# corenel/pytorch-glow

Measured on AMD Instinct MI355X. Metric: images/sec full Glow fwd+logdet, 64x64x3 L=3 K=32, 1/2/4/8 GPU, higher is better.
Workload: dtype f32 (2xf16 split operands, fp32 accumulate); 1 GPU; CelebA 64x64x3 Glow L=3 K=32 hidden=512 affine+invconv, fwd+logdet, batch 64/GPU (BASELINE configs[1]); global_batch=64, parallelism=dp1, repack_every_step=True

## Files before the change

pytorch-glow_amd/csrc/pack.hip:

```cpp
#include <algorithm>

#include "kernels.h"
#include "conv_mfma.h"
#include "sh.h"
#include "lu_wave.h"

namespace glowhip {

__device__ __forceinline__ size_t align_up_dev(size_t v, size_t a) { return (v + a - 1) / a * a; }

__device__ __forceinline__ void pack_scales(const ScaleJob& j, char* packed, int bx, int nbx) {
    float* scale = (float*)(packed + j.scale_off);
    float* inv = j.has_inv ? (float*)(packed + j.inv_off) : nullptr;
    for (int i = bx * 256 + threadIdx.x; i < j.n; i += nbx * 256) {
        const float l3 = j.logs[i] * LOGSCALE;
        scale[i] = expf(l3);
        if (inv) inv[i] = expf(-l3);
    }
}
__global__ void __launch_bounds__(256) k_pack_scales_batched(const ScaleJob* __restrict__ jobs, char* packed) {
    pack_scales(jobs[blockIdx.y], packed, blockIdx.x, gridDim.x);
}

__device__ __forceinline__ void repack_legacy(const RepackJob& j, char* packed, int bx, int nbx) {
    float* out = (float*)(packed + j.out_off);
    if (j.kind == REPACK_WIDE) {
        const long total = (long)j.Kpad * j.Cout;
        for (long e = (long)bx * 256 + threadIdx.x; e < total; e += (long)nbx * 256) {
            const int k = (int)(e / j.Cout), o = (int)(e - (long)k * j.Cout);
            out[e] = (k < j.K) ? j.w[(long)o * j.K + k] : 0.f;
        }
    } else if (j.kind == REPACK_FIRST) {
        const long total = (long)9 * j.Cin * j.Cout;
        for (long e = (long)bx * 256 + threadIdx.x; e < total; e += (long)nbx * 256) {
            const int o = (int)(e % j.Cout);
            const int k = (int)(e / j.Cout);
            const int chunk = k / 54, r = k - chunk * 54;
            const int tap = r / 6, cl = r - tap * 6;
            const int ci = chunk * 6 + cl;
            const float wv = j.transposed ? j.w[((long)ci * j.Cout + o) * 9 + (8 - tap)] : j.w[((long)o * j.Cin + ci) * 9 + tap];
            out[e] = j.fold_logs ? wv * expf(j.fold_logs[o] * LOGSCALE) : wv;
        }
        for (long o = (long)bx * 256 + threadIdx.x; o < j.Cout; o += (long)nbx * 256)
            out[total + o] = j.fold_logs ? j.fold_bias[o] * expf(j.fold_logs[o] * LOGSCALE) : 0.f;
    } else {
        for (long e = (long)bx * 256 + threadIdx.x; e < j.total; e += (long)nbx * 256) {
            const int i = (int)(e & 15), kq = (int)((e >> 4) & 3);
            long t = e >> 6;
            const int mt = (int)(t % j.MT); t /= j.MT;
            const int tap = (int)(t % 9); t /= 9;
            const int c4 = (int)(t % (TAIL_CK / 4));
            const int chunk = (int)(t / (TAIL_CK / 4));
            const int ci = chunk * TAIL_CK + c4 * 4 + kq;
            const int o = tail_row_channel(mt * 16 + i, j.Cout, j.paired);
            out[e] = (o >= 0 && ci < j.Cin)
                         ? (j.transposed ? j.w[((long)ci * j.Cout + o) * 9 + (8 - tap)] : j.w[((long)o * j.Cin + ci) * 9 + tap])
                         : 0.f;
        }
    }
}
__global__ void __launch_bounds__(256) k_repack_batched(const RepackJob* __restrict__ jobs, char* packed) {
    const RepackJob j = jobs[blockIdx.y];
    if (j.kind >= REPACK_SH2_GEMM) return;
    repack_legacy(j, packed, blockIdx.x, gridDim.x);
}

__device__ __forceinline__ const float* repack_src(const RepackJob& j, const char* packed) {
    return j.w ? j.w : reinterpret_cast<const float*>(packed + j.w_off);
}

template <int KIND>
__device__ __forceinline__ void repack_sh2_rows(const RepackJob& j, char* packed, int bx, int nbx) {
    const float* jw = repack_src(j, packed);
    const int lane = threadIdx.x & 63, r8 = lane & 7, gl = lane >> 3;
    const int M = KIND == REPACK_SH2_TAIL ? j.Kpad : j.Cout;
    const int Kp = KIND == REPACK_SH2_FIRST ? j.K * 8 : j.Cin;
    const int ngroups = Kp / 8;
    _Float16* oh = (_Float16*)(packed + j.out_off);
    float* rowscale = (float*)(packed + j.out_off + (size_t)2 * Kp * M * sizeof(_Float16));
    float* rbias = rowscale + M;
    const int nchunk = (j.Cin + 7) / 8;
    for (int r0 = (bx * 4 + (threadIdx.x >> 6)) * 8; r0 < M; r0 += nbx * 32) {
        const int r = r0 + r8;
        const bool rv = r < M;
        float fold = 1.f;
        if (rv && KIND != REPACK_SH2_TAIL && j.fold_logs) fold = expf(j.fold_logs[r] * LOGSCALE);
        auto group = [&](int gi, float (&v)[8]) {
#pragma unroll
            for (int k8 = 0; k8 < 8; ++k8) v[k8] = 0.f;
            if (!rv || gi >= ngroups) return;
            if (KIND == REPACK_SH2_GEMM) {
                const float* src = jw + (long)r * j.Cin + (j.kperm ? sh2_kperm_src(gi * 8) : gi * 8);
                const int h2o = j.kperm ? 8 : 4;
                if ((j.Cin & 3) == 0) {
                    const f32x4_t a = *reinterpret_cast<const f32x4_t*>(src), b = *reinterpret_cast<const f32x4_t*>(src + h2o);
#pragma unroll
                    for (int k8 = 0; k8 < 4; ++k8) { v[k8] = a[k8] * fold; v[4 + k8] = b[k8] * fold; }
                } else {
#pragma unroll
                    for (int k8 = 0; k8 < 8; ++k8) v[k8] = src[(k8 & 3) + (k8 >> 2) * h2o] * fold;
                }
            } else if (KIND == REPACK_SH2_FIRST) {
                const int ch = gi / 9, tap = gi - ch * 9;
                if (ch < nchunk) {
#pragma unroll
                    for (int k8 = 0; k8 < 8; ++k8)
                        if (ch * 8 + k8 < j.Cin) v[k8] = jw[((long)r * j.Cin + ch * 8 + k8) * 9 + tap] * fold;
                }
            } else if (r < 9 * j.Cout) {
                const int tap = r / j.Cout, co = r - tap * j.Cout;
#pragma unroll
                for (int k8 = 0; k8 < 8; ++k8) v[k8] = jw[((long)co * j.Cin + gi * 8 + k8) * 9 + tap];
            }
        };
        float mx = 0.f;
        for (int gi = gl; gi < ngroups; gi += 8) {
            float v[8];
            group(gi, v);
#pragma unroll
            for (int k8 = 0; k8 < 8; ++k8) mx = fmaxf(mx, fabsf(v[k8]));
        }
        mx = fmaxf(mx, __shfl_xor(mx, 8, 64));
        mx = fmaxf(mx, __shfl_xor(mx, 16, 64));
        mx = fmaxf(mx, __shfl_xor(mx, 32, 64));
        int e = 0;
        if (mx > 0.f && mx < 3.0e38f) {
            int ex;
            (void)frexpf(mx, &ex);
            e = 13 - ex;
            e = e > 100 ? 100 : (e < -100 ? -100 : e);
        }
        const float up = ldexpf(1.f, e);
        for (int gi = gl; gi < ngroups; gi += 8) {
            float v[8];
            group(gi, v);
            h8 hi, lo;
#pragma unroll
            for (int k8 = 0; k8 < 8; ++k8) {
                _Float16 a, b;
                sh2_split(v[k8] * up, a, b);
                hi[k8] = a; lo[k8] = b;
            }
            if (rv) {
                *reinterpret_cast<h8*>(oh + ((long)gi * M + r) * 8) = hi;
                *reinterpret_cast<h8*>(oh + ((long)(ngroups + gi) * M + r) * 8) = lo;
            }
        }
        if (gl == 0 && rv) {
            if (KIND == REPACK_SH2_TAIL) {
                rowscale[r] = ldexpf(1.f, -e) * SH2_ACT_INV;
                rbias[r] = 0.f;
            } else {
                rowscale[r] = ldexpf(1.f, -e);
                rbias[r] = (j.fold_bias ? j.fold_bias[r] * fold : 0.f) * SH2_ACT_SCALE;
            }
        }
    }
}

__device__ __forceinline__ void load_brick(const float* src, int nk, bool valid, float (&b)[72]) {
#pragma unroll
    for (int i = 0; i < 72; ++i) b[i] = 0.f;
    if (!valid) return;
    const int count = nk * 9;
    if (nk == 8 && ((size_t)src & 15) == 0) {
#pragma unroll
        for (int i = 0; i < 18; ++i) {
            const f32x4_t v = reinterpret_cast<const f32x4_t*>(src)[i];
#pragma unroll
            for (int q = 0; q < 4; ++q) b[i * 4 + q] = v[q];
        }
    } else if ((count & 1) == 0 && ((size_t)src & 7) == 0) {
#pragma unroll
        for (int i = 0; i < 36; ++i)
            if (2 * i < count) {
                const f32x2_t v = reinterpret_cast<const f32x2_t*>(src)[i];
                b[2 * i] = v[0]; b[2 * i + 1] = v[1];
            }
    } else {
#pragma unroll
        for (int i = 0; i < 72; ++i)
            if (i < count) b[i] = src[i];
    }
}

__device__ __forceinline__ int sh2_row_exponent(float mx) {
    int e = 0;
    if (mx > 0.f && mx < 3.0e38f) {
        int ex;
        (void)frexpf(mx, &ex);
        e = 13 - ex;
        e = e > 100 ? 100 : (e < -100 ? -100 : e);
    }
    return e;
}

__device__ __forceinline__ void brick_emit(const float (&b)[72], int tap, float mul, h8& hi, h8& lo) {
#pragma unroll
    for (int k8 = 0; k8 < 8; ++k8) {
        _Float16 x, y;
        sh2_split(b[k8 * 9 + tap] * mul, x, y);
        hi[k8] = x; lo[k8] = y;
    }
}

__device__ __forceinline__ void repack_sh2_first(const RepackJob& j, char* packed, int bx, int nbx) {
    const int M = j.Cout, G = j.K, Kp = G * 8;
    _Float16* oh = (_Float16*)(packed + j.out_off);
    float* rowscale = (float*)(packed + j.out_off + (size_t)2 * Kp * M * sizeof(_Float16));
    float* rbias = rowscale + M;
    const int nchunk = (j.Cin + 7) / 8;
    for (int r = bx * 256 + threadIdx.x; r < M; r += nbx * 256) {
        const float fold = j.fold_logs ? expf(j.fold_logs[r] * LOGSCALE) : 1.f;
        const float* row = repack_src(j, packed) + (long)r * j.Cin * 9;
        float mx = 0.f;
        for (int ch = 0; ch < nchunk; ++ch) {
            float b[72];
            load_brick(row + ch * 72, min(8, j.Cin - ch * 8), true, b);
#pragma unroll
            for (int i = 0; i < 72; ++i) mx = fmaxf(mx, fabsf(b[i] * fold));
        }
        const int e = sh2_row_exponent(mx);
        const float up = ldexpf(1.f, e);
        for (int ch = 0; ch < nchunk; ++ch) {
            float b[72];
            load_brick(row + ch * 72, min(8, j.Cin - ch * 8), true, b);
#pragma unroll
            for (int i = 0; i < 72; ++i) b[i] *= fold;
#pragma unroll
            for (int tap = 0; tap < 9; ++tap) {
                h8 hi, lo;
                brick_emit(b, tap, up, hi, lo);
                const int gi = ch * 9 + tap;
                *reinterpret_cast<h8*>(oh + ((long)gi * M + r) * 8) = hi;
                *reinterpret_cast<h8*>(oh + ((long)(G + gi) * M + r) * 8) = lo;
            }
        }
        h8 z;
#pragma unroll
        for (int k8 = 0; k8 < 8; ++k8) z[k8] = (_Float16)0.f;
        for (int gi = nchunk * 9; gi < G; ++gi) {
            *reinterpret_cast<h8*>(oh + ((long)gi * M + r) * 8) = z;
            *reinterpret_cast<h8*>(oh + ((long)(G + gi) * M + r) * 8) = z;
        }
        rowscale[r] = ldexpf(1.f, -e);
        rbias[r] = (j.fold_bias ? j.fold_bias[r] * fold : 0.f) * SH2_ACT_SCALE;
    }
}

__device__ __forceinline__ void repack_sh2_first_wide(const RepackJob& j, char* packed, int bx, int nbx) {
    const int M = j.Cout, G = j.K, Kp = G * 8;
    _Float16* oh = (_Float16*)(packed + j.out_off);
    float* rowscale = (float*)(packed + j.out_off + (size_t)2 * Kp * M * sizeof(_Float16));
    float* rbias = rowscale + M;
    const int nchunk = (j.Cin + 7) / 8;
    const int lane = threadIdx.x & 63, r8 = lane & 7, gl = lane >> 3;
    for (int r0 = (bx * 4 + (threadIdx.x >> 6)) * 8; r0 < M; r0 += nbx * 32) {
        const int r = r0 + r8;
        const bool rv = r < M;
        const float fold = (rv && j.fold_logs) ? expf(j.fold_logs[r] * LOGSCALE) : 1.f;
        const float* row = repack_src(j, packed) + (long)(rv ? r : 0) * j.Cin * 9;
        float mx = 0.f;
        for (int ch = gl; ch < nchunk; ch += 8) {
            float b[72];
            load_brick(row + ch * 72, min(8, j.Cin - ch * 8), rv, b);
#pragma unroll
            for (int i = 0; i < 72; ++i) mx = fmaxf(mx, fabsf(b[i] * fold));
        }
        mx = fmaxf(mx, __shfl_xor(mx, 8, 64));
        mx = fmaxf(mx, __shfl_xor(mx, 16, 64));
        mx = fmaxf(mx, __shfl_xor(mx, 32, 64));
        const int e = sh2_row_exponent(mx);
        const float up = ldexpf(1.f, e);
        for (int ch = gl; ch < nchunk; ch += 8) {
            float b[72];
            load_brick(row + ch * 72, min(8, j.Cin - ch * 8), rv, b);
#pragma unroll
            for (int i = 0; i < 72; ++i) b[i] *= fold;
            if (!rv) continue;
#pragma unroll
            for (int tap = 0; tap < 9; ++tap) {
                h8 hi, lo;
                brick_emit(b, tap, up, hi, lo);
                const int gi = ch * 9 + tap;
                *reinterpret_cast<h8*>(oh + ((long)gi * M + r) * 8) = hi;
                *reinterpret_cast<h8*>(oh + ((long)(G + gi) * M + r) * 8) = lo;
            }
        }
        if (!rv) continue;
        h8 z;
#pragma unroll
        for (int k8 = 0; k8 < 8; ++k8) z[k8] = (_Float16)0.f;
        for (int gi = nchunk * 9 + gl; gi < G; gi += 8) {
            *reinterpret_cast<h8*>(oh + ((long)gi * M + r) * 8) = z;
            *reinterpret_cast<h8*>(oh + ((long)(G + gi) * M + r) * 8) = z;
        }
        if (gl == 0) {
            rowscale[r] = ldexpf(1.f, -e);
            rbias[r] = (j.fold_bias ? j.fold_bias[r] * fold : 0.f) * SH2_ACT_SCALE;
        }
    }
}

__device__ __forceinline__ void load_brick_kperm(const float* row, int gi, bool valid, float (&b)[72]) {
#pragma unroll
    for (int i = 0; i < 72; ++i) b[i] = 0.f;
    if (!valid) return;
    const int k0 = sh2_kperm_src(gi * 8);
    const float* s0 = row + (long)k0 * 9;
    const float* s1 = row + (long)(k0 + 8) * 9;
    if ((((size_t)s0 | (size_t)s1) & 15) == 0) {
#pragma unroll
        for (int i = 0; i < 9; ++i) {
            const f32x4_t v = reinterpret_cast<const f32x4_t*>(s0)[i], w = reinterpret_cast<const f32x4_t*>(s1)[i];
#pragma unroll
            for (int q = 0; q < 4; ++q) { b[i * 4 + q] = v[q]; b[36 + i * 4 + q] = w[q]; }
        }
    } else {
#pragma unroll
        for (int i = 0; i < 36; ++i) { b[i] = s0[i]; b[36 + i] = s1[i]; }
    }
}

__device__ __forceinline__ void repack_sh2_tail(const RepackJob& j, char* packed, int bx, int nbx) {
    __shared__ float s_mx[4][9][8];
    const int lane = threadIdx.x & 63, wave = threadIdx.x >> 6, r8 = lane & 7, gl = lane >> 3;
    const int M = j.Kpad, Kp = j.Cin, ngroups = Kp / 8, rows = 9 * j.Cout;
    _Float16* oh = (_Float16*)(packed + j.out_off);
    float* rowscale = (float*)(packed + j.out_off + (size_t)2 * Kp * M * sizeof(_Float16));
    float* rbias = rowscale + M;
    for (int co0 = bx * 8; co0 < j.Cout; co0 += nbx * 8) {
        const int co = co0 + r8;
        const bool rv = co < j.Cout;
        const float* row = repack_src(j, packed) + (long)(rv ? co : 0) * j.Cin * 9;
        float mx[9];
#pragma unroll
        for (int t = 0; t < 9; ++t) mx[t] = 0.f;
        for (int gi = wave * 8 + gl; gi < ngroups; gi += 32) {
            float b[72];
            if (j.kperm) load_brick_kperm(row, gi, rv, b); else load_brick(row + gi * 72, 8, rv, b);
#pragma unroll
            for (int t = 0; t < 9; ++t)
#pragma unroll
                for (int k8 = 0; k8 < 8; ++k8) mx[t] = fmaxf(mx[t], fabsf(b[k8 * 9 + t]));
        }
#pragma unroll
        for (int t = 0; t < 9; ++t) {
            mx[t] = fmaxf(mx[t], __shfl_xor(mx[t], 8, 64));
            mx[t] = fmaxf(mx[t], __shfl_xor(mx[t], 16, 64));
            mx[t] = fmaxf(mx[t], __shfl_xor(mx[t], 32, 64));
            if (gl == 0) s_mx[wave][t][r8] = mx[t];
        }
        __syncthreads();
        int e[9];
#pragma unroll
        for (int t = 0; t < 9; ++t)
            e[t] = sh2_row_exponent(fmaxf(fmaxf(s_mx[0][t][r8], s_mx[1][t][r8]), fmaxf(s_mx[2][t][r8], s_mx[3][t][r8])));
        __syncthreads();
        for (int gi = wave * 8 + gl; gi < ngroups; gi += 32) {
            float b[72];
            if (j.kperm) load_brick_kperm(row, gi, rv, b); else load_brick(row + gi * 72, 8, rv, b);
            if (rv) {
#pragma unroll
                for (int t = 0; t < 9; ++t) {
                    h8 hi, lo;
                    brick_emit(b, t, ldexpf(1.f, e[t]), hi, lo);
                    const int r = t * j.Cout + co;
                    *reinterpret_cast<h8*>(oh + ((long)gi * M + r) * 8) = hi;
                    *reinterpret_cast<h8*>(oh + ((long)(ngroups + gi) * M + r) * 8) = lo;
                }
            }
        }
        if (wave == 0 && gl == 0 && rv) {
#pragma unroll
            for (int t = 0; t < 9; ++t) {
                rowscale[t * j.Cout + co] = ldexpf(1.f, -e[t]) * SH2_ACT_INV;
                rbias[t * j.Cout + co] = 0.f;
            }
        }
    }
    const int pad = M - rows;
    h8 z;
#pragma unroll
    for (int k8 = 0; k8 < 8; ++k8) z[k8] = (_Float16)0.f;
    for (int el = bx * 256 + threadIdx.x; el < pad * 2 * ngroups; el += nbx * 256) {
        const int g2 = el / pad, r = rows + (el - g2 * pad);
        *reinterpret_cast<h8*>(oh + ((long)g2 * M + r) * 8) = z;
    }
    for (int r = rows + bx * 256 + threadIdx.x; r < M; r += nbx * 256) {
        rowscale[r] = SH2_ACT_INV;
        rbias[r] = 0.f;
    }
}

template <int KIND>
__global__ void __launch_bounds__(256) k_repack_sh2_batched(const RepackJob* __restrict__ jobs, char* packed) {
    const RepackJob j = jobs[blockIdx.y];
    if (j.kind != KIND) return;
    const int bx = blockIdx.x, nbx = gridDim.x;
    if (KIND == REPACK_SH2_GEMM) repack_sh2_rows<REPACK_SH2_GEMM>(j, packed, bx, nbx);
    else if (KIND == REPACK_SH2_FIRST) { if (j.Cin >= 64) repack_sh2_first_wide(j, packed, bx, nbx); else repack_sh2_first(j, packed, bx, nbx); }
    else repack_sh2_tail(j, packed, bx, nbx);
}

__global__ void __launch_bounds__(256) k_pack_fused(const PackSeg* __restrict__ segs, const StepPrepJob* __restrict__ prep, int n_prep,
                                                    const RepackJob* __restrict__ rjobs, const ScaleJob* __restrict__ sjobs,
                                                    unsigned* counter, int n_lu_blocks, char* packed) {
    const PackSeg sg = segs[blockIdx.x];
    switch (sg.kind) {
    case PACKSEG_LU: {
        __shared__ double v[256];
        __shared__ int s_last;
        step_prepare_small_body(prep, n_prep, packed, sg.bx);
        __threadfence();
        __syncthreads();
        if (threadIdx.x == 0) {
            const unsigned old = __hip_atomic_fetch_add(counter, 1u, __ATOMIC_RELAXED, __HIP_MEMORY_SCOPE_AGENT);
            s_last = old + 1 == (unsigned)n_lu_blocks;
            if (s_last) __hip_atomic_store(counter, 0u, __ATOMIC_RELAXED, __HIP_MEMORY_SCOPE_AGENT);
        }
        __syncthreads();
        if (!s_last) break;
        __threadfence();
        double t = 0.0;
        for (int base = 0; base < n_prep; base += 256) {
            const int i = base + threadIdx.x;
            v[threadIdx.x] = i < n_prep ? __hip_atomic_load((const double*)(packed + prep[i].konst_off), __ATOMIC_RELAXED, __HIP_MEMORY_SCOPE_AGENT) : 0.0;
            __syncthreads();
            if (threadIdx.x == 0)
                for (int q = 0; q < 256 && base + q < n_prep; ++q) t += v[q];
            __syncthreads();
        }
        if (threadIdx.x == 0) *(double*)packed = t;
        break;
    }
    case PACKSEG_SH2_GEMM: repack_sh2_rows<REPACK_SH2_GEMM>(rjobs[sg.job], packed, sg.bx, sg.nbx); break;
    case PACKSEG_SH2_FIRST: {
        const RepackJob j = rjobs[sg.job];
        if (j.Cin >= 64) repack_sh2_first_wide(j, packed, sg.bx, sg.nbx); else repack_sh2_first(j, packed, sg.bx, sg.nbx);
        break;
    }
    case PACKSEG_SH2_TAIL: repack_sh2_tail(rjobs[sg.job], packed, sg.bx, sg.nbx); break;
    case PACKSEG_LEGACY: repack_legacy(rjobs[sg.job], packed, sg.bx, sg.nbx); break;
    case PACKSEG_SCALE: pack_scales(sjobs[sg.job], packed, sg.bx, sg.nbx); break;
    default:
        if (threadIdx.x < 64 && (threadIdx.x >= 2 || n_prep == 0)) reinterpret_cast<float*>(packed)[threadIdx.x] = 0.f;
        break;
    }
}

int pack_fused_job_blocks(int seg_kind, const RepackJob* r, const ScaleJob* sj) {
    switch (seg_kind) {
    case PACKSEG_SH2_GEMM: return std::max(1, (r->Cout + 31) / 32);
    case PACKSEG_SH2_FIRST: return std::max(1, r->Cin >= 64 ? std::min(16, (r->Cout + 31) / 32) : (r->Cout + 255) / 256);
    case PACKSEG_SH2_TAIL: return std::max(1, (r->Cout + 7) / 8);
    case PACKSEG_LEGACY: {
        const long total = r->kind == REPACK_WIDE ? (long)r->Kpad * r->Cout : (r->kind == REPACK_FIRST ? (long)9 * r->Cin * r->Cout : r->total);
        return (int)std::max(1L, std::min(64L, (total + 255) / 256));
    }
    case PACKSEG_SCALE: return std::max(1, std::min(2, (sj->n + 255) / 256));
    default: return 1;
    }
}

int launch_pack_fused(const PackSeg* segs_dev, int n_segs, const StepPrepJob* prep_dev, int n_prep, const RepackJob* rj_dev,
                      const ScaleJob* sj_dev, unsigned* counter_dev, void* packed, hipStream_t s) {
    hipLaunchKernelGGL(k_pack_fused, dim3(n_segs), dim3(256), 0, s, segs_dev, prep_dev, n_prep, rj_dev, sj_dev, counter_dev,
                       (n_prep + 3) / 4, (char*)packed);
    GH_LAUNCH_CHECK("k_pack_fused");
    return GLOWHIP_OK;
}

__global__ void __launch_bounds__(256) k_flipT_batched(const FlipJob* __restrict__ jobs, char* packed, int first, int stride) {
    __shared__ float tile[32][32 * 9 + 1];
    const FlipJob j = jobs[first + blockIdx.y * stride];
    const int ti = (j.I + 31) / 32, to = (j.O + 31) / 32;
    if ((int)blockIdx.x >= ti * to) return;
    const int o0 = (blockIdx.x / ti) * 32, i0 = (blockIdx.x % ti) * 32;
    const int ks = j.ks, run = 32 * ks;
    float* dst = reinterpret_cast<float*>(packed + j.dst_off);
    for (int e = threadIdx.x; e < 32 * run; e += 256) {
        const int ol = e / run, r = e - ol * run;
        const int o = o0 + ol, i = i0 + r / ks;
        tile[ol][r] = (o < j.O && i < j.I) ? j.src[((long)o * j.I + i0) * ks + r] : 0.f;
    }
    __syncthreads();
    for (int e = threadIdx.x; e < 32 * run; e += 256) {
        const int il = e / run, r = e - il * run;
        const int ol = r / ks, tap = r - ol * ks;
        const int i = i0 + il, o = o0 + ol;
        if (i < j.I && o < j.O) dst[((long)i * j.O + o0) * ks + r] = tile[ol][il * ks + (ks - 1 - tap)];
    }
}

int launch_flipT_batched(const FlipJob* jobs_dev, int n_jobs, const int* max_tiles3, void* packed, hipStream_t s) {
    if (n_jobs == 0) return GLOWHIP_OK;
    GH_REQUIRE(n_jobs % 3 == 0, "flipT: jobs come in triples");
    for (int k = 0; k < 3; ++k) {
        hipLaunchKernelGGL(k_flipT_batched, dim3(std::max(1, max_tiles3[k]), n_jobs / 3), dim3(256), 0, s, jobs_dev, (char*)packed, k, 3);
        GH_LAUNCH_CHECK("k_flipT_batched");
    }
    return GLOWHIP_OK;
}

int launch_pack_batched(const ScaleJob* sj_dev, int n_scale, const RepackJob* rj_dev, const int* n_kind, int tail_blocks, void* packed,
                        hipStream_t s, hipStream_t s_legacy, int first_blocks) {
    if (n_scale > 0) {
// ... 28 lines not shown
```

pytorch-glow_amd/csrc/plan_build.hip:

```cpp
#include "plan_internal.h"

namespace glowhip {

static int hip_failed(const char* what) { set_error("%s", what); return GLOWHIP_ELAUNCH; }

struct Fold { const float* bias = nullptr; const float* logs = nullptr; };
static RepackJob& add_job(glowhip_plan* p, int kind, const float* w, size_t w_off, size_t out_off, int Cin, int Cout, Fold fold, int use) {
    RepackJob r{};
    r.kind = kind; r.w = w; r.w_off = w_off; r.out_off = out_off; r.Cin = Cin; r.Cout = Cout; r.fold_bias = fold.bias; r.fold_logs = fold.logs; r.use = use;
    p->repack_jobs.push_back(r);
    return p->repack_jobs.back();
}
static void add_wide(glowhip_plan* p, const float* w, size_t out_off, int Cin, int Cout, int ksize, int use) {
    RepackJob& r = add_job(p, REPACK_WIDE, w, 0, out_off, Cin, Cout, Fold{}, use);
    r.K = Cin * ksize * ksize; r.Kpad = wide_kpad(Cin, ksize);
}
static void add_tail(glowhip_plan* p, const float* w, size_t out_off, int Cin, int Cout, int paired, int transposed, int use) {
    RepackJob& r = add_job(p, REPACK_TAIL, w, 0, out_off, Cin, Cout, Fold{}, use);
    r.paired = paired; r.MT = tail_mt(Cout, paired); r.total = (long)tail_chunks(Cin) * (TAIL_CK / 4) * 9 * r.MT * 64; r.transposed = transposed;
}
static void add_first(glowhip_plan* p, const float* w, size_t out_off, int Cin, int Cout, Fold fold, int transposed, int use) {
    add_job(p, REPACK_FIRST, w, 0, out_off, Cin, Cout, fold, use).transposed = transposed;
}
static void add_sh2_gemm(glowhip_plan* p, const float* w, size_t w_off, size_t out_off, int Cin, int Cout, Fold fold, int kperm, int after_lu, int use) {
// ... 141 lines not shown
        p->flip_jobs.push_back(FlipJob{d.f4_w, L.wt4, L.Cout, hid, 9});
        p->flip_jobs.push_back(FlipJob{d.f2_w, L.wt2, hid, hid, 1});
        p->flip_jobs.push_back(FlipJob{d.f0_w, L.wt0, hid, Ch, 9});
        const int th = (hid + 31) / 32;
        p->flip_tiles[0] = std::max(p->flip_tiles[0], th * ((L.Cout + 31) / 32));
        p->flip_tiles[1] = std::max(p->flip_tiles[1], th * th);
        p->flip_tiles[2] = std::max(p->flip_tiles[2], th * ((Ch + 31) / 32));
        add_sh2_first(p, nullptr, L.wt4, L.cb_w0, L.Cout, hid, Fold{nullptr, d.f2_an_logs}, TRAIN);
        add_sh2_gemm(p, nullptr, L.wt2, L.cb_w2, hid, hid, Fold{nullptr, d.f0_an_logs},  1,  0, TRAIN);
        add_sh2_tail(p, nullptr, L.wt0, L.cb_w4, hid, Ch, TRAIN);
    }
    if (L.mfma_last) add_tail(p, d.f4_w, L.f4_wp, hid, L.Cout,  d.coupling == GLOWHIP_COUPLING_AFFINE,  0, fp32);
    if (L.wide_last) add_wide(p, d.f4_w, L.f4_wt, hid, L.Cout,  3, fp32);
    if (L.dg4_first) add_first(p, d.f4_w, L.f4T_wf, L.Cout, hid, Fold{},  1, TRAIN);
    if (L.dg0_tail) add_tail(p, d.f0_w, L.f0T_wp, hid, Ch,  0,  1, TRAIN);
}
static void split_jobs(glowhip_plan* p, const LayerPlan& L) {
    p->scale_jobs.push_back(ScaleJob{L.d.f4_logs, L.f4_scale, 0, L.Cout, 0});
    if (L.mfma_last) add_tail(p, L.d.f4_w, L.f4_wp, L.d.C / 2, L.Cout,  1,  0, GLOWHIP_PACK_INFERENCE | GLOWHIP_PACK_TRAINING);
}
static void lu_widths(glowhip_plan* p) {
    p->max_lds_c = p->max_c = 0;
    for (const StepPrepJob& j : p->prep_jobs)
        if (j.w) { p->max_c = std::max(p->max_c, j.C); if (j.C <= 64) p->max_lds_c = std::max(p->max_lds_c, j.C); }
}

static int seg_kind(const RepackJob& r) { return r.kind < REPACK_SH2_GEMM ? PACKSEG_LEGACY : PACKSEG_SH2_GEMM + (r.kind - REPACK_SH2_GEMM); }
static void layout_tables(glowhip_plan* p, size_t& off) {
    p->prep_off = take(off, p->prep_jobs.size() * sizeof(StepPrepJob));
    p->scale_off = take(off, p->scale_jobs.size() * sizeof(ScaleJob));
    p->repack_off = take(off, REPACK_SLOTS * p->repack_jobs.size() * sizeof(RepackJob));
    p->flip_off = take(off, p->flip_jobs.size() * sizeof(FlipJob));
    size_t n_inv = 0;
    for (const StepPrepJob& pj : p->prep_jobs) n_inv += pj.w ? 1 : 0;
    p->lu_off = take(off, n_inv * sizeof(LuJob));
    size_t nseg = (p->prep_jobs.size() + 3) / 4 + 1;
    for (const RepackJob& r : p->repack_jobs) nseg += pack_fused_job_blocks(seg_kind(r), &r, nullptr);
    for (const ScaleJob& sj : p->scale_jobs) nseg += pack_fused_job_blocks(PACKSEG_SCALE, nullptr, &sj);
    p->seg_cap = nseg;
    p->seg_off = take(off, PACK_SEG_HEAD + nseg * sizeof(PackSeg));
}

struct PackSel { int n_kind[5] = {0, 0, 0, 0, 0}, tail_blocks = 1, first_blocks = 2; };
static PackSel select_jobs(glowhip_plan* plan, int use) {
    PackSel sel;
    plan->repack_sel.clear();
    auto group = [](const RepackJob& r) { return r.after_lu ? 4 : (r.kind < REPACK_SH2_GEMM ? 0 : r.kind - REPACK_SH2_GEMM + 1); };
    for (int gk = 0; gk < 5; ++gk)
        for (const RepackJob& r : plan->repack_jobs)
            if ((r.use & use) && group(r) == gk) {
                plan->repack_sel.push_back(r);
                ++sel.n_kind[gk];
                if (gk == 3) sel.tail_blocks = std::max(sel.tail_blocks, (r.Cout + 7) / 8);
                if (gk == 2 && r.Cin >= 64) sel.first_blocks = std::max(sel.first_blocks, std::min(16, (r.Cout + 31) / 32));
            }
    return sel;
}

static bool upload(void* packed, size_t off, const void* src, size_t bytes, hipStream_t s) {
    return bytes == 0 || hipMemcpyAsync((char*)packed + off, src, bytes, hipMemcpyHostToDevice, s) == hipSuccess;
}
static int send_tables(glowhip_plan* plan, void* packed, int slot, size_t slot_off, hipStream_t s) {
    if (plan->tables_in != packed) {
        if (!upload(packed, plan->prep_off, plan->prep_jobs.data(), plan->prep_jobs.size() * sizeof(StepPrepJob), s) ||
            !upload(packed, plan->scale_off, plan->scale_jobs.data(), plan->scale_jobs.size() * sizeof(ScaleJob), s) ||
            !upload(packed, plan->flip_off, plan->flip_jobs.data(), plan->flip_jobs.size() * sizeof(FlipJob), s) ||
            !upload(packed, plan->lu_off, plan->lu_jobs.data(), plan->lu_jobs.size() * sizeof(LuJob), s))
            return hip_failed("plan_pack: hipMemcpyAsync of the job tables failed");
        plan->tables_in = packed; plan->slots_in = 0; plan->segs_in = false;
    }
    if (!(plan->slots_in & (1u << slot))) {
        std::vector<RepackJob>& keep = plan->repack_slot_host[slot];
        keep = plan->repack_sel;
        if (!upload(packed, slot_off, keep.data(), keep.size() * sizeof(RepackJob), s))
            return hip_failed("plan_pack: hipMemcpyAsync of the repack job table failed");
        plan->slots_in |= 1u << slot;
    }
    return GLOWHIP_OK;
}
static void build_segments(glowhip_plan* plan, const PackSel& sel) {
    std::vector<PackSeg>& t = plan->pack_segs;
    t.clear();
    auto add = [&t](int kind, int jn, int nb) { for (int b = 0; b < nb; ++b) t.push_back(PackSeg{kind, jn, b, nb}); };
    auto add_repack = [&](int jn) { const RepackJob& r = plan->repack_sel[jn]; add(seg_kind(r), jn, pack_fused_job_blocks(seg_kind(r), &r, nullptr)); };
    for (int b = 0; b < ((int)plan->prep_jobs.size() + 3) / 4; ++b) t.push_back(PackSeg{PACKSEG_LU, 0, b, 1});
    for (int jn = sel.n_kind[0]; jn < (int)plan->repack_sel.size(); ++jn) add_repack(jn);
    for (int jn = 0; jn < sel.n_kind[0]; ++jn) add_repack(jn);
    for (int jn = 0; jn < (int)plan->scale_jobs.size(); ++jn) add(PACKSEG_SCALE, jn, pack_fused_job_blocks(PACKSEG_SCALE, nullptr, &plan->scale_jobs[jn]));
    add(PACKSEG_ZERO, 0, 1);
}
static int send_segments(glowhip_plan* plan, void* packed, const PackSel& sel, int slot, hipStream_t s) {
    GH_REQUIRE(sel.n_kind[4] == 0, "plan_pack: the one-launch pack takes no W^-1 image");
    if (plan->pack_segs.empty() || plan->pack_segs_slot != slot) {
        build_segments(plan, sel);
        plan->pack_segs_slot = slot; plan->segs_in = false;
    }
    GH_REQUIRE(plan->pack_segs.size() <= plan->seg_cap, "plan_pack: segment table larger than its slot");
    if (plan->segs_in) return GLOWHIP_OK;
    static const char zero_head[PACK_SEG_HEAD] = {0};
    if (!upload(packed, plan->seg_off, zero_head, PACK_SEG_HEAD, s) ||
        !upload(packed, plan->seg_off + PACK_SEG_HEAD, plan->pack_segs.data(), plan->pack_segs.size() * sizeof(PackSeg), s))
        return hip_failed("plan_pack: hipMemcpyAsync of the segment table failed");
    plan->segs_in = true;
    return GLOWHIP_OK;
}
static int fork_side(glowhip_plan* plan, hipStream_t s, hipStream_t* side) {
    *side = s;
// ... 175 lines not shown
```

Baseline: 9574 images/sec.

## Stage repack weight rows in LDS and hold bricks across the two repack passes

The SH2 repack kernels used to read every weight brick from global memory twice, once to find the row max-abs exponent and again to emit the hi/lo f16 split. They now keep the first brick in registers and park a second brick in a shared-memory stage buffer, and the GEMM repack copies rows into swizzled LDS with deep-unrolled loads. The small-Cin first-layer repack now spreads channel chunks across waves, with an LDS max reduction and more blocks. This costs a 72KB shared buffer per block, added syncthreads and a launch_bounds occupancy hint, all to cut redundant global reads in the per-step repack.

```diff
diff --git a/pytorch-glow_amd/csrc/pack.hip b/pytorch-glow_amd/csrc/pack.hip
--- a/pytorch-glow_amd/csrc/pack.hip
+++ b/pytorch-glow_amd/csrc/pack.hip
@@ -65,52 +65,87 @@
     repack_legacy(j, packed, blockIdx.x, gridDim.x);
 }
 
-__device__ __forceinline__ const float* repack_src(const RepackJob& j, const char* packed) {
-    return j.w ? j.w : reinterpret_cast<const float*>(packed + j.w_off);
-}
-
-template <int KIND>
-__device__ __forceinline__ void repack_sh2_rows(const RepackJob& j, char* packed, int bx, int nbx) {
-    const float* jw = repack_src(j, packed);
-    const int lane = threadIdx.x & 63, r8 = lane & 7, gl = lane >> 3;
-    const int M = KIND == REPACK_SH2_TAIL ? j.Kpad : j.Cout;
-    const int Kp = KIND == REPACK_SH2_FIRST ? j.K * 8 : j.Cin;
-    const int ngroups = Kp / 8;
+typedef __attribute__((address_space(1))) const float gfloat;
+typedef __attribute__((address_space(1))) const f32x2_t gf32x2;
+typedef __attribute__((address_space(1))) const f32x4_t gf32x4;
+__device__ __forceinline__ gfloat* repack_src(const RepackJob& j, const char* packed) {
+    return (gfloat*)(j.w ? j.w : reinterpret_cast<const float*>(packed + j.w_off));
+}
+
+__device__ __forceinline__ int sh2_row_exponent(float mx) {
+    int e = 0;
+    if (mx > 0.f && mx < 3.0e38f) {
+        int ex;
+        (void)frexpf(mx, &ex);
+        e = 13 - ex;
+        e = e > 100 ? 100 : (e < -100 ? -100 : e);
+    }
+    return e;
+}
+
+constexpr int SH2_STAGE_K = 512;
+constexpr int SH2_STAGE_LD = SH2_STAGE_K + 64;
+constexpr int SH2_STAGE_FLOATS = 256 * 72;
+static_assert(32 * SH2_STAGE_LD <= SH2_STAGE_FLOATS, "SH2_GEMM stages 32 rows");
+__device__ __forceinline__ int sh2_stage_swz(int row) { return 32 * (row & 1) + 8 * ((row >> 1) & 1); }
+
+template <typename V, int U, typename Src, typename Dst>
+__device__ __forceinline__ void sh2_stage_wave(int count, int lane, Src src, Dst dst) {
+    for (int f0 = 0; f0 < count; f0 += U * 64) {
+        V v[U];
+#pragma unroll
+        for (int u = 0; u < U; ++u) v[u] = *src(min(f0 + u * 64 + lane, count - 1));
+#pragma unroll
+        for (int u = 0; u < U; ++u)
+            if (f0 + u * 64 + lane < count) *dst(f0 + u * 64 + lane) = v[u];
+    }
+}
+template <typename V, typename Src, typename Dst>
+__device__ __forceinline__ void sh2_stage(int count, int lane, Src src, Dst dst) {
+    const int deep = count / (16 * 64) * (16 * 64);
+    sh2_stage_wave<V, 16>(deep, lane, src, dst);
+    sh2_stage_wave<V, 4>(count - deep, lane, [&](int f) { return src(deep + f); }, [&](int f) { return dst(deep + f); });
+}
+
+__device__ __forceinline__ void repack_sh2_rows(const RepackJob& j, char* packed, int bx, int nbx, float* stage) {
+    const gfloat* jw = repack_src(j, packed);
+    const int lane = threadIdx.x & 63, wave = __builtin_amdgcn_readfirstlane(threadIdx.x >> 6), r8 = lane & 7, gl = lane >> 3;
+    const int M = j.Cout, Kp = j.Cin, ngroups = Kp / 8;
     _Float16* oh = (_Float16*)(packed + j.out_off);
     float* rowscale = (float*)(packed + j.out_off + (size_t)2 * Kp * M * sizeof(_Float16));
     float* rbias = rowscale + M;
-    const int nchunk = (j.Cin + 7) / 8;
-    for (int r0 = (bx * 4 + (threadIdx.x >> 6)) * 8; r0 < M; r0 += nbx * 32) {
-        const int r = r0 + r8;
+    const int gk = j.kperm ? 32 : 8, h2o = j.kperm ? 8 : 4;
+    const int kst = min(Kp, SH2_STAGE_K) / gk * gk;
+    float* srow = stage + (wave * 8 + r8) * SH2_STAGE_LD + sh2_stage_swz(r8);
+    for (int rb = bx * 32; rb < M; rb += nbx * 32) {
+        const int r0 = rb + wave * 8, r = r0 + r8;
         const bool rv = r < M;
+        if ((Kp & 3) == 0 && ((size_t)jw & 15) == 0) {
+            const int k4 = kst / 4;
+            sh2_stage<f32x4_t>(8 * k4, lane,
+                [&](int f) { const int row = f / k4; return reinterpret_cast<const gf32x4*>(jw + (long)min(r0 + row, M - 1) * Kp + (f - row * k4) * 4); },
+                [&](int f) { const int row = f / k4; return reinterpret_cast<f32x4_t*>(stage + (wave * 8 + row) * SH2_STAGE_LD + sh2_stage_swz(row) + (f - row * k4) * 4); });
+        } else {
+            sh2_stage<float>(8 * kst, lane,
+                [&](int f) { const int row = f / kst; return jw + (long)min(r0 + row, M - 1) * Kp + (f - row * kst); },
+                [&](int f) { const int row = f / kst; return stage + (wave * 8 + row) * SH2_STAGE_LD + sh2_stage_swz(row) + (f - row * kst); });
+        }
+        __syncthreads();
         float fold = 1.f;
-        if (rv && KIND != REPACK_SH2_TAIL && j.fold_logs) fold = expf(j.fold_logs[r] * LOGSCALE);
+        if (rv && j.fold_logs) fold = expf(j.fold_logs[r] * LOGSCALE);
         auto group = [&](int gi, float (&v)[8]) {
 #pragma unroll
             for (int k8 = 0; k8 < 8; ++k8) v[k8] = 0.f;
             if (!rv || gi >= ngroups) return;
-            if (KIND == REPACK_SH2_GEMM) {
-                const float* src = jw + (long)r * j.Cin + (j.kperm ? sh2_kperm_src(gi * 8) : gi * 8);
-                const int h2o = j.kperm ? 8 : 4;
-                if ((j.Cin & 3) == 0) {
-                    const f32x4_t a = *reinterpret_cast<const f32x4_t*>(src), b = *reinterpret_cast<const f32x4_t*>(src + h2o);
-#pragma unroll
-                    for (int k8 = 0; k8 < 4; ++k8) { v[k8] = a[k8] * fold; v[4 + k8] = b[k8] * fold; }
-                } else {
-#pragma unroll
-                    for (int k8 = 0; k8 < 8; ++k8) v[k8] = src[(k8 & 3) + (k8 >> 2) * h2o] * fold;
-                }
-            } else if (KIND == REPACK_SH2_FIRST) {
-                const int ch = gi / 9, tap = gi - ch * 9;
-                if (ch < nchunk) {
-#pragma unroll
-                    for (int k8 = 0; k8 < 8; ++k8)
-                        if (ch * 8 + k8 < j.Cin) v[k8] = jw[((long)r * j.Cin + ch * 8 + k8) * 9 + tap] * fold;
-                }
-            } else if (r < 9 * j.Cout) {
-                const int tap = r / j.Cout, co = r - tap * j.Cout;
-#pragma unroll
-                for (int k8 = 0; k8 < 8; ++k8) v[k8] = jw[((long)co * j.Cin + gi * 8 + k8) * 9 + tap];
+            const int k0 = j.kperm ? sh2_kperm_src(gi * 8) : gi * 8;
+            if ((gi * 8 / gk + 1) * gk <= kst) {
+                const f32x4_t a = *reinterpret_cast<const f32x4_t*>(srow + k0), b = *reinterpret_cast<const f32x4_t*>(srow + k0 + h2o);
+#pragma unroll
+                for (int k8 = 0; k8 < 4; ++k8) { v[k8] = a[k8] * fold; v[4 + k8] = b[k8] * fold; }
+            } else {
+                const gfloat* src = jw + (long)r * Kp + k0;
+#pragma unroll
+                for (int k8 = 0; k8 < 8; ++k8) v[k8] = src[(k8 & 3) + (k8 >> 2) * h2o] * fold;
             }
         };
         float mx = 0.f;
@@ -123,13 +158,7 @@
         mx = fmaxf(mx, __shfl_xor(mx, 8, 64));
         mx = fmaxf(mx, __shfl_xor(mx, 16, 64));
         mx = fmaxf(mx, __shfl_xor(mx, 32, 64));
-        int e = 0;
-        if (mx > 0.f && mx < 3.0e38f) {
-            int ex;
-            (void)frexpf(mx, &ex);
-            e = 13 - ex;
-            e = e > 100 ? 100 : (e < -100 ? -100 : e);
-        }
+        const int e = sh2_row_exponent(mx);
         const float up = ldexpf(1.f, e);
         for (int gi = gl; gi < ngroups; gi += 8) {
             float v[8];
@@ -147,34 +176,31 @@
             }
         }
         if (gl == 0 && rv) {
-            if (KIND == REPACK_SH2_TAIL) {
-                rowscale[r] = ldexpf(1.f, -e) * SH2_ACT_INV;
-                rbias[r] = 0.f;
-            } else {
-                rowscale[r] = ldexpf(1.f, -e);
-                rbias[r] = (j.fold_bias ? j.fold_bias[r] * fold : 0.f) * SH2_ACT_SCALE;
-            }
-        }
-    }
-}
-
-__device__ __forceinline__ void load_brick(const float* src, int nk, bool valid, float (&b)[72]) {
-#pragma unroll
-    for (int i = 0; i < 72; ++i) b[i] = 0.f;
-    if (!valid) return;
+            rowscale[r] = ldexpf(1.f, -e);
+            rbias[r] = (j.fold_bias ? j.fold_bias[r] * fold : 0.f) * SH2_ACT_SCALE;
+        }
+        __syncthreads();
+    }
+}
+
+__device__ __forceinline__ void load_brick(const gfloat* src, int nk, float (&b)[72]) {
     const int count = nk * 9;
     if (nk == 8 && ((size_t)src & 15) == 0) {
 #pragma unroll
         for (int i = 0; i < 18; ++i) {
-            const f32x4_t v = reinterpret_cast<const f32x4_t*>(src)[i];
+            const f32x4_t v = reinterpret_cast<const gf32x4*>(src)[i];
 #pragma unroll
             for (int q = 0; q < 4; ++q) b[i * 4 + q] = v[q];
         }
-    } else if ((count & 1) == 0 && ((size_t)src & 7) == 0) {
+        return;
+    }
+#pragma unroll
+    for (int i = 0; i < 72; ++i) b[i] = 0.f;
+    if ((count & 1) == 0 && ((size_t)src & 7) == 0) {
 #pragma unroll
         for (int i = 0; i < 36; ++i)
             if (2 * i < count) {
-                const f32x2_t v = reinterpret_cast<const f32x2_t*>(src)[i];
+                const f32x2_t v = reinterpret_cast<const gf32x2*>(src)[i];
                 b[2 * i] = v[0]; b[2 * i + 1] = v[1];
             }
     } else {
@@ -184,15 +210,19 @@
     }
 }
 
-__device__ __forceinline__ int sh2_row_exponent(float mx) {
-    int e = 0;
-    if (mx > 0.f && mx < 3.0e38f) {
-        int ex;
-        (void)frexpf(mx, &ex);
-        e = 13 - ex;
-        e = e > 100 ? 100 : (e < -100 ? -100 : e);
-    }
-    return e;
+__device__ __forceinline__ void brick_to_stage(float* stage, const float (&b)[72]) {
+    f32x4_t* s = reinterpret_cast<f32x4_t*>(stage) + threadIdx.x;
+#pragma unroll
+    for (int q = 0; q < 18; ++q) s[q * 256] = f32x4_t{b[4 * q], b[4 * q + 1], b[4 * q + 2], b[4 * q + 3]};
+}
+__device__ __forceinline__ void brick_from_stage(const float* stage, float (&b)[72]) {
+    const f32x4_t* s = reinterpret_cast<const f32x4_t*>(stage) + threadIdx.x;
+#pragma unroll
+    for (int q = 0; q < 18; ++q) {
+        const f32x4_t v = s[q * 256];
+#pragma unroll
+        for (int i = 0; i < 4; ++i) b[4 * q + i] = v[i];
+    }
 }
 
 __device__ __forceinline__ void brick_emit(const float (&b)[72], int tap, float mul, h8& hi, h8& lo) {
@@ -204,51 +234,74 @@
     }
 }
 
-__device__ __forceinline__ void repack_sh2_first(const RepackJob& j, char* packed, int bx, int nbx) {
+__device__ __forceinline__ void first_emit(float (&b)[72], float fold, float up, _Float16* oh, int ch, int G, int M, int r) {
+#pragma unroll
+    for (int i = 0; i < 72; ++i) b[i] *= fold;
+#pragma unroll
+    for (int tap = 0; tap < 9; ++tap) {
+        h8 hi, lo;
+        brick_emit(b, tap, up, hi, lo);
+        const int gi = ch * 9 + tap;
+        *reinterpret_cast<h8*>(oh + ((long)gi * M + r) * 8) = hi;
+        *reinterpret_cast<h8*>(oh + ((long)(G + gi) * M + r) * 8) = lo;
+        __builtin_amdgcn_sched_barrier(0);
+    }
+}
+
+__device__ __forceinline__ void repack_sh2_first(const RepackJob& j, char* packed, int bx, int nbx, float* stage) {
+    __shared__ float s_mx[4][64];
+    const int lane = threadIdx.x & 63, wave = __builtin_amdgcn_readfirstlane(threadIdx.x >> 6);
     const int M = j.Cout, G = j.K, Kp = G * 8;
     _Float16* oh = (_Float16*)(packed + j.out_off);
     float* rowscale = (float*)(packed + j.out_off + (size_t)2 * Kp * M * sizeof(_Float16));
     float* rbias = rowscale + M;
     const int nchunk = (j.Cin + 7) / 8;
-    for (int r = bx * 256 + threadIdx.x; r < M; r += nbx * 256) {
-        const float fold = j.fold_logs ? expf(j.fold_logs[r] * LOGSCALE) : 1.f;
-        const float* row = repack_src(j, packed) + (long)r * j.Cin * 9;
+    const bool has0 = wave < nchunk, has1 = wave + 4 < nchunk;
+    for (int rb = bx * 64; rb < M; rb += nbx * 64) {
+        const int r = rb + lane, rc = min(r, M - 1);
+        const bool rv = r < M;
+        const float fold = j.fold_logs ? expf(j.fold_logs[rc] * LOGSCALE) : 1.f;
+        const gfloat* row = repack_src(j, packed) + (long)rc * j.Cin * 9;
+        float held[72];
         float mx = 0.f;
-        for (int ch = 0; ch < nchunk; ++ch) {
+        if (has1) {
             float b[72];
-            load_brick(row + ch * 72, min(8, j.Cin - ch * 8), true, b);
+            load_brick(row + (wave + 4) * 72, min(8, j.Cin - (wave + 4) * 8), b);
 #pragma unroll
             for (int i = 0; i < 72; ++i) mx = fmaxf(mx, fabsf(b[i] * fold));
-        }
-        const int e = sh2_row_exponent(mx);
+            brick_to_stage(stage, b);
+        }
+        if (has0) {
+            load_brick(row + wave * 72, min(8, j.Cin - wave * 8), held);
+#pragma unroll
+            for (int i = 0; i < 72; ++i) mx = fmaxf(mx, fabsf(held[i] * fold));
+        }
+        s_mx[wave][lane] = mx;
+        __syncthreads();
+        const int e = sh2_row_exponent(fmaxf(fmaxf(s_mx[0][lane], s_mx[1][lane]), fmaxf(s_mx[2][lane], s_mx[3][lane])));
         const float up = ldexpf(1.f, e);
-        for (int ch = 0; ch < nchunk; ++ch) {
+        if (has0 && rv) first_emit(held, fold, up, oh, wave, G, M, r);
+        if (has1) {
             float b[72];
-            load_brick(row + ch * 72, min(8, j.Cin - ch * 8), true, b);
-#pragma unroll
-            for (int i = 0; i < 72; ++i) b[i] *= fold;
-#pragma unroll
-            for (int tap = 0; tap < 9; ++tap) {
-                h8 hi, lo;
-                brick_emit(b, tap, up, hi, lo);
-                const int gi = ch * 9 + tap;
-                *reinterpret_cast<h8*>(oh + ((long)gi * M + r) * 8) = hi;
-                *reinterpret_cast<h8*>(oh + ((long)(G + gi) * M + r) * 8) = lo;
-            }
+            brick_from_stage(stage, b);
+            if (rv) first_emit(b, fold, up, oh, wave + 4, G, M, r);
         }
         h8 z;
 #pragma unroll
         for (int k8 = 0; k8 < 8; ++k8) z[k8] = (_Float16)0.f;
-        for (int gi = nchunk * 9; gi < G; ++gi) {
+        for (int gi = nchunk * 9 + wave; gi < G && rv; gi += 4) {
             *reinterpret_cast<h8*>(oh + ((long)gi * M + r) * 8) = z;
             *reinterpret_cast<h8*>(oh + ((long)(G + gi) * M + r) * 8) = z;
         }
-        rowscale[r] = ldexpf(1.f, -e);
-        rbias[r] = (j.fold_bias ? j.fold_bias[r] * fold : 0.f) * SH2_ACT_SCALE;
-    }
-}
-
-__device__ __forceinline__ void repack_sh2_first_wide(const RepackJob& j, char* packed, int bx, int nbx) {
+        if (wave == 0 && rv) {
+            rowscale[r] = ldexpf(1.f, -e);
+            rbias[r] = (j.fold_bias ? j.fold_bias[r] * fold : 0.f) * SH2_ACT_SCALE;
+        }
+        __syncthreads();
+    }
+}
+
+__device__ __forceinline__ void repack_sh2_first_wide(const RepackJob& j, char* packed, int bx, int nbx, float* stage) {
     const int M = j.Cout, G = j.K, Kp = G * 8;
     _Float16* oh = (_Float16*)(packed + j.out_off);
     float* rowscale = (float*)(packed + j.out_off + (size_t)2 * Kp * M * sizeof(_Float16));
@@ -259,33 +312,29 @@
         const int r = r0 + r8;
         const bool rv = r < M;
         const float fold = (rv && j.fold_logs) ? expf(j.fold_logs[r] * LOGSCALE) : 1.f;
-        const float* row = repack_src(j, packed) + (long)(rv ? r : 0) * j.Cin * 9;
+        const gfloat* row = repack_src(j, packed) + (long)min(r, M - 1) * j.Cin * 9;
+        float held[72];
+        load_brick(row + gl * 72, min(8, j.Cin - gl * 8), held);
         float mx = 0.f;
-        for (int ch = gl; ch < nchunk; ch += 8) {
+#pragma unroll
+        for (int i = 0; i < 72; ++i) mx = fmaxf(mx, fabsf(held[i] * fold));
+        for (int ch = gl + 8; ch < nchunk; ch += 8) {
             float b[72];
-            load_brick(row + ch * 72, min(8, j.Cin - ch * 8), rv, b);
+            load_brick(row + ch * 72, min(8, j.Cin - ch * 8), b);
 #pragma unroll
             for (int i = 0; i < 72; ++i) mx = fmaxf(mx, fabsf(b[i] * fold));
+            if (ch == gl + 8) brick_to_stage(stage, b);
         }
         mx = fmaxf(mx, __shfl_xor(mx, 8, 64));
         mx = fmaxf(mx, __shfl_xor(mx, 16, 64));
         mx = fmaxf(mx, __shfl_xor(mx, 32, 64));
         const int e = sh2_row_exponent(mx);
         const float up = ldexpf(1.f, e);
-        for (int ch = gl; ch < nchunk; ch += 8) {
+        if (rv) first_emit(held, fold, up, oh, gl, G, M, r);
+        for (int ch = gl + 8; ch < nchunk; ch += 8) {
             float b[72];
-            load_brick(row + ch * 72, min(8, j.Cin - ch * 8), rv, b);
-#pragma unroll
-            for (int i = 0; i < 72; ++i) b[i] *= fold;
-            if (!rv) continue;
-#pragma unroll
-            for (int tap = 0; tap < 9; ++tap) {
-                h8 hi, lo;
-                brick_emit(b, tap, up, hi, lo);
-                const int gi = ch * 9 + tap;
-                *reinterpret_cast<h8*>(oh + ((long)gi * M + r) * 8) = hi;
-                *reinterpret_cast<h8*>(oh + ((long)(G + gi) * M + r) * 8) = lo;
-            }
+            if (ch == gl + 8) brick_from_stage(stage, b); else load_brick(row + ch * 72, min(8, j.Cin - ch * 8), b);
+            if (rv) first_emit(b, fold, up, oh, ch, G, M, r);
         }
         if (!rv) continue;
         h8 z;
@@ -302,17 +351,14 @@
     }
 }
 
-__device__ __forceinline__ void load_brick_kperm(const float* row, int gi, bool valid, float (&b)[72]) {
-#pragma unroll
-    for (int i = 0; i < 72; ++i) b[i] = 0.f;
-    if (!valid) return;
+__device__ __forceinline__ void load_brick_kperm(const gfloat* row, int gi, float (&b)[72]) {
     const int k0 = sh2_kperm_src(gi * 8);
-    const float* s0 = row + (long)k0 * 9;
-    const float* s1 = row + (long)(k0 + 8) * 9;
+    const gfloat* s0 = row + (long)k0 * 9;
+    const gfloat* s1 = row + (long)(k0 + 8) * 9;
     if ((((size_t)s0 | (size_t)s1) & 15) == 0) {
 #pragma unroll
         for (int i = 0; i < 9; ++i) {
-            const f32x4_t v = reinterpret_cast<const f32x4_t*>(s0)[i], w = reinterpret_cast<const f32x4_t*>(s1)[i];
+            const f32x4_t v = reinterpret_cast<const gf32x4*>(s0)[i], w = reinterpret_cast<const gf32x4*>(s1)[i];
 #pragma unroll
             for (int q = 0; q < 4; ++q) { b[i * 4 + q] = v[q]; b[36 + i * 4 + q] = w[q]; }
         }
@@ -322,9 +368,9 @@
     }
 }
 
-__device__ __forceinline__ void repack_sh2_tail(const RepackJob& j, char* packed, int bx, int nbx) {
+__device__ __forceinline__ void repack_sh2_tail(const RepackJob& j, char* packed, int bx, int nbx, float* stage) {
     __shared__ float s_mx[4][9][8];
-    const int lane = threadIdx.x & 63, wave = threadIdx.x >> 6, r8 = lane & 7, gl = lane >> 3;
+    const int lane = threadIdx.x & 63, wave = __builtin_amdgcn_readfirstlane(threadIdx.x >> 6), r8 = lane & 7, gl = lane >> 3;
     const int M = j.Kpad, Kp = j.Cin, ngroups = Kp / 8, rows = 9 * j.Cout;
     _Float16* oh = (_Float16*)(packed + j.out_off);
     float* rowscale = (float*)(packed + j.out_off + (size_t)2 * Kp * M * sizeof(_Float16));
@@ -332,17 +378,34 @@
     for (int co0 = bx * 8; co0 < j.Cout; co0 += nbx * 8) {
         const int co = co0 + r8;
         const bool rv = co < j.Cout;
-        const float* row = repack_src(j, packed) + (long)(rv ? co : 0) * j.Cin * 9;
+        const gfloat* row = repack_src(j, packed) + (long)min(co, j.Cout - 1) * j.Cin * 9;
         float mx[9];
 #pragma unroll
         for (int t = 0; t < 9; ++t) mx[t] = 0.f;
-        for (int gi = wave * 8 + gl; gi < ngroups; gi += 32) {
+        auto fetch = [&](int gi, float (&b)[72]) {
+            if (j.kperm) load_brick_kperm(row, gi, b); else load_brick(row + gi * 72, 8, b);
+#pragma unroll
+            for (int t = 0; t < 9; ++t)
+#pragma unroll
+                for (int k8 = 0; k8 < 8; ++k8) mx[t] = fmaxf(mx[t], fabsf(b[k8 * 9 + t]));
+        };
+        auto emit = [&](int gi, const float (&b)[72], const int (&e)[9]) {
+#pragma unroll
+            for (int t = 0; t < 9; ++t) {
+                h8 hi, lo;
+                brick_emit(b, t, ldexpf(1.f, e[t]), hi, lo);
+                const int r = t * j.Cout + co;
+                *reinterpret_cast<h8*>(oh + ((long)gi * M + r) * 8) = hi;
+                *reinterpret_cast<h8*>(oh + ((long)(ngroups + gi) * M + r) * 8) = lo;
+            }
+        };
+        const int g0 = wave * 8 + gl;
+        float held[72];
+        fetch(min(g0, ngroups - 1), held);
+        for (int gi = g0 + 32; gi < ngroups; gi += 32) {
             float b[72];
-            if (j.kperm) load_brick_kperm(row, gi, rv, b); else load_brick(row + gi * 72, 8, rv, b);
-#pragma unroll
-            for (int t = 0; t < 9; ++t)
-#pragma unroll
-                for (int k8 = 0; k8 < 8; ++k8) mx[t] = fmaxf(mx[t], fabsf(b[k8 * 9 + t]));
+            fetch(gi, b);
+            if (gi == g0 + 32) brick_to_stage(stage, b);
         }
 #pragma unroll
         for (int t = 0; t < 9; ++t) {
@@ -357,19 +420,12 @@
         for (int t = 0; t < 9; ++t)
             e[t] = sh2_row_exponent(fmaxf(fmaxf(s_mx[0][t][r8], s_mx[1][t][r8]), fmaxf(s_mx[2][t][r8], s_mx[3][t][r8])));
         __syncthreads();
-        for (int gi = wave * 8 + gl; gi < ngroups; gi += 32) {
+        if (rv && g0 < ngroups) emit(g0, held, e);
+        for (int gi = g0 + 32; gi < ngroups; gi += 32) {
             float b[72];
-            if (j.kperm) load_brick_kperm(row, gi, rv, b); else load_brick(row + gi * 72, 8, rv, b);
-            if (rv) {
-#pragma unroll
-                for (int t = 0; t < 9; ++t) {
-                    h8 hi, lo;
-                    brick_emit(b, t, ldexpf(1.f, e[t]), hi, lo);
-                    const int r = t * j.Cout + co;
-                    *reinterpret_cast<h8*>(oh + ((long)gi * M + r) * 8) = hi;
-                    *reinterpret_cast<h8*>(oh + ((long)(ngroups + gi) * M + r) * 8) = lo;
-                }
-            }
+            if (gi == g0 + 32) brick_from_stage(stage, b);
+            else if (j.kperm) load_brick_kperm(row, gi, b); else load_brick(row + gi * 72, 8, b);
+            if (rv) emit(gi, b, e);
         }
         if (wave == 0 && gl == 0 && rv) {
 #pragma unroll
@@ -394,18 +450,20 @@
 }
 
 template <int KIND>
-__global__ void __launch_bounds__(256) k_repack_sh2_batched(const RepackJob* __restrict__ jobs, char* packed) {
+__global__ void __launch_bounds__(256, 2) k_repack_sh2_batched(const RepackJob* __restrict__ jobs, char* packed) {
     const RepackJob j = jobs[blockIdx.y];
     if (j.kind != KIND) return;
+    __shared__ __attribute__((aligned(16))) float stage[SH2_STAGE_FLOATS];
     const int bx = blockIdx.x, nbx = gridDim.x;
-    if (KIND == REPACK_SH2_GEMM) repack_sh2_rows<REPACK_SH2_GEMM>(j, packed, bx, nbx);
-    else if (KIND == REPACK_SH2_FIRST) { if (j.Cin >= 64) repack_sh2_first_wide(j, packed, bx, nbx); else repack_sh2_first(j, packed, bx, nbx); }
-    else repack_sh2_tail(j, packed, bx, nbx);
-}
-
-__global__ void __launch_bounds__(256) k_pack_fused(const PackSeg* __restrict__ segs, const StepPrepJob* __restrict__ prep, int n_prep,
+    if (KIND == REPACK_SH2_GEMM) repack_sh2_rows(j, packed, bx, nbx, stage);
+    else if (KIND == REPACK_SH2_FIRST) { if (j.Cin >= 64) repack_sh2_first_wide(j, packed, bx, nbx, stage); else repack_sh2_first(j, packed, bx, nbx, stage); }
+    else repack_sh2_tail(j, packed, bx, nbx, stage);
+}
+
+__global__ void __launch_bounds__(256, 2) k_pack_fused(const PackSeg* __restrict__ segs, const StepPrepJob* __restrict__ prep, int n_prep,
                                                     const RepackJob* __restrict__ rjobs, const ScaleJob* __restrict__ sjobs,
                                                     unsigned* counter, int n_lu_blocks, char* packed) {
+    __shared__ __attribute__((aligned(16))) float stage[SH2_STAGE_FLOATS];
     const PackSeg sg = segs[blockIdx.x];
     switch (sg.kind) {
     case PACKSEG_LU: {
@@ -434,13 +492,13 @@
         if (threadIdx.x == 0) *(double*)packed = t;
         break;
     }
-    case PACKSEG_SH2_GEMM: repack_sh2_rows<REPACK_SH2_GEMM>(rjobs[sg.job], packed, sg.bx, sg.nbx); break;
+    case PACKSEG_SH2_GEMM: repack_sh2_rows(rjobs[sg.job], packed, sg.bx, sg.nbx, stage); break;
     case PACKSEG_SH2_FIRST: {
         const RepackJob j = rjobs[sg.job];
-        if (j.Cin >= 64) repack_sh2_first_wide(j, packed, sg.bx, sg.nbx); else repack_sh2_first(j, packed, sg.bx, sg.nbx);
+        if (j.Cin >= 64) repack_sh2_first_wide(j, packed, sg.bx, sg.nbx, stage); else repack_sh2_first(j, packed, sg.bx, sg.nbx, stage);
         break;
     }
-    case PACKSEG_SH2_TAIL: repack_sh2_tail(rjobs[sg.job], packed, sg.bx, sg.nbx); break;
+    case PACKSEG_SH2_TAIL: repack_sh2_tail(rjobs[sg.job], packed, sg.bx, sg.nbx, stage); break;
     case PACKSEG_LEGACY: repack_legacy(rjobs[sg.job], packed, sg.bx, sg.nbx); break;
     case PACKSEG_SCALE: pack_scales(sjobs[sg.job], packed, sg.bx, sg.nbx); break;
     default:
@@ -452,7 +510,7 @@
 int pack_fused_job_blocks(int seg_kind, const RepackJob* r, const ScaleJob* sj) {
     switch (seg_kind) {
     case PACKSEG_SH2_GEMM: return std::max(1, (r->Cout + 31) / 32);
-    case PACKSEG_SH2_FIRST: return std::max(1, r->Cin >= 64 ? std::min(16, (r->Cout + 31) / 32) : (r->Cout + 255) / 256);
+    case PACKSEG_SH2_FIRST: return std::max(1, r->Cin >= 64 ? std::min(16, (r->Cout + 31) / 32) : std::min(16, (r->Cout + 63) / 64));
     case PACKSEG_SH2_TAIL: return std::max(1, (r->Cout + 7) / 8);
     case PACKSEG_LEGACY: {
         const long total = r->kind == REPACK_WIDE ? (long)r->Kpad * r->Cout : (r->kind == REPACK_FIRST ? (long)9 * r->Cin * r->Cout : r->total);
diff --git a/pytorch-glow_amd/csrc/plan_build.hip b/pytorch-glow_amd/csrc/plan_build.hip
--- a/pytorch-glow_amd/csrc/plan_build.hip
+++ b/pytorch-glow_amd/csrc/plan_build.hip
@@ -217,7 +217,7 @@
                 plan->repack_sel.push_back(r);
                 ++sel.n_kind[gk];
                 if (gk == 3) sel.tail_blocks = std::max(sel.tail_blocks, (r.Cout + 7) / 8);
-                if (gk == 2 && r.Cin >= 64) sel.first_blocks = std::max(sel.first_blocks, std::min(16, (r.Cout + 31) / 32));
+                if (gk == 2) sel.first_blocks = std::max(sel.first_blocks, pack_fused_job_blocks(PACKSEG_SH2_FIRST, &r, nullptr));
             }
     return sel;
 }
```

Result: no change. 9645 images/sec, median of 6 (+0.7%).
